# teticio/audio-diffusion

Hardware: NVIDIA H100
Metric: mel-spectrograms/sec (1000-step DDPM, 256x256x1) (higher is better)
Workload: dtype bf16 operands, fp32 accumulate (fp32 master weights, fp64 GroupNorm sums)

## Files before the change

### audio_diffusion_b200/csrc/conv_tc.cu

```cuda
#include <cuda.h>
#include <cudaTypedefs.h>

#include <cstdlib>

#include "conv_tc.cuh"

namespace b200ad {

struct alignas(64) ConvMaps {
  CUtensorMap src[CONV_MAXSEG];
  CUtensorMap out;
};

__host__ __device__ __forceinline__ int window_pixels(const ConvParams& p, const ConvSeg& sg, int G) {
  return p.tile2d ? (p.tw + sg.hl + sg.hr) * (p.th + sg.ht + sg.hb)
                  : G * CONV_TM + (sg.ht + sg.hb) * p.Wp + sg.hl + sg.hr;
}
__host__ __device__ __forceinline__ int window_pitch(const ConvParams& p, const ConvSeg& sg) {
  return p.tile2d ? p.tw + sg.hl + sg.hr : p.Wp;
}

constexpr int CONV_THREADS = 384;
constexpr int CONV_XF_THREADS = 64;
constexpr int CONV_SPLANE = CONV_MAXG * CONV_TM * 16;
constexpr int CONV_STG_WG = 8 * CONV_SPLANE;
constexpr int CONV_STAGING = 2 * CONV_STG_WG;
static size_t conv_smem_bytes(const ConvParams& p) {
  return (size_t)p.as * p.a_stage + (size_t)p.bs * CONV_B_SLOT + CONV_STAGING + 1024;
}

struct WorkItem {
  int n, ntile, m0, G;
  int r0, c0;
};

__device__ __forceinline__ WorkItem decode_work(const ConvParams& p, int w) {
  WorkItem wi;
  wi.ntile = w % p.ntiles_n;
  const int gidx = w / p.ntiles_n;
  if (p.tile2d) {
    wi.n = gidx / p.groups_per_img;
    const int t = gidx - wi.n * p.groups_per_img, tx = t / p.tiles_y;
    wi.r0 = (t - tx * p.tiles_y) * p.th;
    wi.c0 = tx * p.tw;
    wi.m0 = 0;
    wi.G = CONV_MAXG;
    return wi;
  }
  wi.r0 = wi.c0 = 0;
  if (p.pack) {
    wi.n = gidx * p.pack;
    wi.m0 = 0;
    wi.G = min(p.pack, p.N - wi.n);
    return wi;
  }
  wi.n = gidx / p.groups_per_img;
  const int g = gidx - wi.n * p.groups_per_img;
  wi.m0 = g * (CONV_MAXG * CONV_TM);
  const int rem = p.H * p.Wp - wi.m0;
  wi.G = min(CONV_MAXG, (rem + CONV_TM - 1) / CONV_TM);
  return wi;
}

template <bool SILU>
__device__ __forceinline__ uint4 xform_vec(uint4 v, const f32x2_t (&sc)[4], const f32x2_t (&sh)[4]) {
  uint32_t u[4] = {v.x, v.y, v.z, v.w};
#pragma unroll
  for (int e = 0; e < 4; ++e) {
    f32x2_t a = f2_fma(f2_from_bf16x2(u[e]), sc[e], sh[e]);
    if (SILU) {
      const float2 f = f2_unpack(a);
      a = f2_fma(a, f2_pack(tanh_approx(f.x), tanh_approx(f.y)), a);
    }
    u[e] = f2_to_bf16x2(a);
  }
  return make_uint4(u[0], u[1], u[2], u[3]);
}

template <bool SQUARE>
__global__ void __launch_bounds__(CONV_THREADS, 1) conv_tc_kernel(const __grid_constant__ ConvParams p,
                                                                  const __grid_constant__ ConvMaps maps) {
  constexpr int ASM = CONV_AS_MAX, BSM = CONV_BS_MAX;
  const int AS = p.as;
  const int BS = p.bs;
  extern __shared__ __align__(128) uint8_t smem[];
  const int warp = __shfl_sync(0xffffffffu, (int)(threadIdx.x >> 5), 0);
  const int lane = threadIdx.x & 31;
  const int a_bytes = p.a_stage;

  uint8_t* bring = smem + AS * a_bytes;
  uint8_t* stg = bring + BS * CONV_B_SLOT;
  uint8_t* ctrl = stg + CONV_STAGING;
  uint64_t* bars = reinterpret_cast<uint64_t*>(ctrl);
  const uint32_t smem_base = smem_u32(smem);
  const uint32_t bring_base = smem_u32(bring);
  const uint32_t bar_fullA = smem_u32(bars);
  const uint32_t bar_readyA = smem_u32(bars + ASM);
  const uint32_t bar_emptyA = smem_u32(bars + 2 * ASM);
  const uint32_t bar_fullB = smem_u32(bars + 3 * ASM);
  const uint32_t bar_emptyB = smem_u32(bars + 3 * ASM + BSM);
  static_assert((3 * ASM + 2 * BSM) * 8 <= 1024, "barrier block overflows");

  if (warp == 1 && lane == 0) {
    for (int s = 0; s < AS; ++s) {
      mbar_init(bar_fullA + 8 * s, 1);
      mbar_init(bar_readyA + 8 * s, CONV_XF_THREADS / 32);
      mbar_init(bar_emptyA + 8 * s, 8);
    }
    for (int s = 0; s < BS; ++s) {
      mbar_init(bar_fullB + 8 * s, 1);
      mbar_init(bar_emptyB + 8 * s, 8);
    }
    mbar_fence_init();
  }
  __syncthreads();

  asm volatile("griddepcontrol.launch_dependents;" ::: "memory");
  if (warp != 1) asm volatile("griddepcontrol.wait;" ::: "memory");

  if (warp == 0) {
    int stage = 0;
    uint32_t phase = 0;
    for (int w = blockIdx.x; w < p.total_work; w += gridDim.x) {
      const WorkItem wi = decode_work(p, w);
      for (int s = 0; s < p.nseg; ++s) {
        const ConvSeg& sg = p.seg[s];
        const uint32_t row_bytes = (uint32_t)window_pixels(p, sg, wi.G) * 16u;
        for (int ks = 0; ks < sg.ksteps; ++ks) {
          const uint32_t full = bar_fullA + 8 * stage;
          if (lane == 0) {
            mbar_wait(bar_emptyA + 8 * stage, phase ^ 1);
            mbar_arrive_expect_tx(full, 2u * row_bytes);
          }
          __syncwarp();
          const long long plane = (long long)(2 * ks + (lane & 1)) * p.PL;
          if (p.tile2d) {
            if (lane == 0)
              tensor_g2s_4d(smem_base + stage * a_bytes, &maps.src[s], 8 * (wi.c0 - sg.hl), wi.r0 - sg.ht, 2 * ks, wi.n, full);
          } else if (!p.pack) {
            const int pix0 = p.lead + wi.m0 - sg.ht * p.Wp - sg.hl;
            if (lane < 2)
              bulk_g2s(smem_base + stage * a_bytes + (uint32_t)lane * row_bytes,
                       sg.src + (long long)wi.n * sg.img_stride + (plane + pix0) * 8, row_bytes, full);
          } else {
            const int g = lane >> 1, lead_px = sg.ht * p.Wp + sg.hl, trail_px = sg.hb * p.Wp + sg.hr;
            const int cnt = CONV_TM + (g == 0 ? lead_px : 0) + (g == wi.G - 1 ? trail_px : 0);
            const int doff = (g == 0) ? 0 : lead_px + g * CONV_TM;
            const int pix0 = p.lead - (g == 0 ? lead_px : 0);
            if (g < wi.G && lane < 2 * CONV_MAXG)
              bulk_g2s(smem_base + stage * a_bytes + (uint32_t)(lane & 1) * row_bytes + (uint32_t)doff * 16u,
                       sg.src + (long long)(wi.n + g) * sg.img_stride + (plane + pix0) * 8, (uint32_t)cnt * 16u, full);
          }
          if (++stage == AS) { stage = 0; phase ^= 1; }
        }
      }
    }
  } else if (warp == 1) {
    if (lane == 0) {
      int stage = 0;
      uint32_t phase = 0;
      for (int w = blockIdx.x; w < p.total_work; w += gridDim.x) {
        const int ntile = w % p.ntiles_n;
        for (int s = 0; s < p.nseg; ++s) {
          const ConvSeg& sg = p.seg[s];
          const char* src = reinterpret_cast<const char*>(sg.wpack + (long long)ntile * sg.wtile_stride);
          for (int ks = 0; ks < sg.ksteps; ++ks) {
            for (int t0 = 0; t0 < sg.ntaps; t0 += CONV_BT) {
              const uint32_t bytes = (uint32_t)min(CONV_BT, sg.ntaps - t0) * CONV_B_TAP;
              mbar_wait(bar_emptyB + 8 * stage, phase ^ 1);
              if (p.dbg & 32) {
                mbar_arrive(bar_fullB + 8 * stage);
              } else {
                mbar_arrive_expect_tx(bar_fullB + 8 * stage, bytes);
                bulk_g2s(bring_base + stage * CONV_B_SLOT, src, bytes, bar_fullB + 8 * stage);
              }
              src += bytes;
              if (++stage == BS) { stage = 0; phase ^= 1; }
            }
          }
        }
      }
    }
  } else if (warp >= 4) {
    const int cw = (warp - 4) >> 2, wq = warp & 3, tid = threadIdx.x & 127;
    const uint32_t stg_w = smem_u32(stg) + (uint32_t)(cw * CONV_STG_WG);
    const uint32_t st_addr = stg_w + (uint32_t)((2 * wq + ((lane >> 3) & 1)) * CONV_SPLANE + (8 * (lane >> 4) + (lane & 7)) * 16);
    const Geom og = make_geom(p.N, p.up2 ? 2 * p.H : p.H, p.up2 ? 2 * p.W : p.W);
    const long long out_img_stride = (long long)(p.cout >> 3) * og.PL * 8;
    const int hw_end = p.H * p.Wp;
    const bool do_stats = p.stats != nullptr;
    const bool issuer = tid < 8 * CONV_MAXG;
    float acc[CONV_MAXG * CONV_TM / 2];
    int sa = 0, sb = 0;
    uint32_t pa = 0, pb = 0;
    for (int w = blockIdx.x; w < p.total_work; w += gridDim.x) {
      const WorkItem wi = decode_work(p, w);
#pragma unroll
      for (int i = 0; i < CONV_MAXG * CONV_TM / 2; ++i) acc[i] = 0.f;
      int pend_b = -1, pend_a = -1;
      auto release = [&]() {
        __syncwarp();
        if (lane == 0) {
          if (pend_b >= 0) mbar_arrive(bar_emptyB + 8 * pend_b);
          if (pend_a >= 0) mbar_arrive(bar_emptyA + 8 * pend_a);
        }
      };
      for (int s = 0, ks = 0; s < p.nseg;) {
        const ConvSeg& sg = p.seg[s];
        const uint32_t xlbo = (uint32_t)window_pixels(p, sg, wi.G) * 16u;
        const uint32_t xsbo = p.tile2d ? (uint32_t)window_pitch(p, sg) * 16u : 128u;
        const int ntaps = sg.ntaps;
        mbar_wait(bar_readyA + 8 * sa, pa);
        const uint32_t abase = smem_base + sa * a_bytes;
        for (int t0 = 0; t0 < ntaps; t0 += CONV_BT) {
          mbar_wait(bar_fullB + 8 * sb, pb);
          const uint32_t bbase = bring_base + sb * CONV_B_SLOT + (uint32_t)(cw * 1024);
          const int nt = min(CONV_BT, ntaps - t0);
          wgmma_fence();
          for (int t = 0; t < nt; ++t) {
            const uint64_t wdesc = gmma_desc(bbase + (uint32_t)t * CONV_B_TAP, (CONV_NT / 8) * 128, 128);
            const uint64_t xdesc = gmma_desc(abase + (uint32_t)sg.aoff[t0 + t] * 16u, xlbo, xsbo);
            if constexpr (SQUARE) {
              wgmma_m64n128k16_x2(acc, wdesc, xdesc, xdesc + (128u >> 4));
            } else if (wi.G == 2) {
              wgmma_m64n256k16<0, 0>(acc, wdesc, xdesc);
            } else {
              wgmma_m64n128k16<0, 0>(acc, wdesc, xdesc);
            }
          }
          wgmma_commit();
          wgmma_wait<1>();
          release();
          pend_b = sb;
          pend_a = (t0 + CONV_BT >= ntaps) ? sa : -1;
          if (++sb == BS) { sb = 0; pb ^= 1; }
        }
        if (++sa == AS) { sa = 0; pa ^= 1; }
        if (++ks == sg.ksteps) { ks = 0; ++s; }
      }
      wgmma_wait<0>();
      release();

      if (issuer) bulk_wait_read_all();
      named_bar_sync(1 + cw, 128);
      if (!(p.dbg & 8)) {
        float ssum[2] = {0.f, 0.f}, ssq[2] = {0.f, 0.f};
#pragma unroll
        for (int g = 0; g < CONV_MAXG; ++g) {
          if (g < wi.G) {
            const int n = p.pack ? wi.n + g : wi.n;
            float bias[2];
#pragma unroll
            for (int h = 0; h < 2; ++h) {
              const int c = wi.ntile * CONV_NT + cw * 64 + wq * 16 + 8 * h + (lane >> 2);
              bias[h] = p.bias ? __ldg(p.bias + c) : 0.f;
              if (p.temb) bias[h] += __ldg(p.temb + (long long)n * p.temb_stride + c);
            }
            int m = (p.pack ? 0 : wi.m0 + g * CONV_TM) + 2 * (lane & 3);
            int col = m % p.Wp;
#pragma unroll
            for (int k = 0; k < CONV_TM / 16; ++k) {
              uint32_t pk[4];
#pragma unroll
              for (int u = 0; u < 2; ++u) {
                const int col1 = (col + 1 == p.Wp) ? 0 : col + 1;
                const bool v0 = p.tile2d || (m < hw_end && col < p.W), v1 = p.tile2d || (m + 1 < hw_end && col1 < p.W);
#pragma unroll
                for (int h = 0; h < 2; ++h) {
                  const int j = g * (CONV_TM / 8) + 2 * k + u;
                  const float a0 = v0 ? acc[4 * j + 2 * h] + bias[h] : 0.f;
                  const float a1 = v1 ? acc[4 * j + 2 * h + 1] + bias[h] : 0.f;
                  ssum[h] += a0 + a1;
                  ssq[h] = fmaf(a0, a0, fmaf(a1, a1, ssq[h]));
                  pk[2 * u + h] = pack_bf16x2(a0, a1);
                }
                m += 8;
                col += 8;
                while (col >= p.Wp) col -= p.Wp;
              }
              stmatrix_x4_trans(st_addr + (uint32_t)((g * CONV_TM + 16 * k) * 16), pk[0], pk[1], pk[2], pk[3]);
            }
            if (do_stats && (p.pack || g == wi.G - 1)) {
#pragma unroll
              for (int h = 0; h < 2; ++h) {
                float s1 = ssum[h], s2 = ssq[h];
#pragma unroll
                for (int o = 1; o < 16; o <<= 1) {
                  s1 += __shfl_xor_sync(0xffffffffu, s1, o);
                  s2 += __shfl_xor_sync(0xffffffffu, s2, o);
                }
                if ((lane & 15) == 0) {
                  const int c = wi.ntile * CONV_NT + cw * 64 + wq * 16 + 8 * h + (lane >> 2);
                  stat_t* sdst = p.stats + ((long long)n * (p.cout >> 2) + (c >> 2)) * 2;
                  atomicAdd(sdst, (stat_t)s1);
                  atomicAdd(sdst + 1, (stat_t)s2);
                }
                ssum[h] = 0.f;
                ssq[h] = 0.f;
              }
            }
          }
        }
      }
      if (p.tile2d) {
        fence_proxy_async_smem();
        named_bar_sync(1 + cw, 128);
        if (SQUARE) {
          const int g = tid >> 3, pl = tid & 7;
          if (issuer && !(p.dbg & 2)) {
            const uint32_t src = stg_w + (uint32_t)(pl * CONV_SPLANE + g * CONV_TM * 16);
            const int c = wi.c0 + 8 * g, plane = wi.ntile * 16 + cw * 8 + pl;
            if (p.up2) tensor_s2g_5d(&maps.out, 0, c, wi.r0, plane, wi.n, src);
            else       tensor_s2g_4d(&maps.out, 8 * c, wi.r0, plane, wi.n, src);
            bulk_commit();
          }
        } else if (tid == 0 && !(p.dbg & 2)) {
          tensor_s2g_4d(&maps.out, 8 * wi.c0, wi.r0, wi.ntile * 16 + cw * 8, wi.n, stg_w);
          bulk_commit();
        }
      } else if (!p.up2) {
        fence_proxy_async_smem();
        named_bar_sync(1 + cw, 128);
        const int g = tid >> 3, pl = tid & 7;
        if (issuer && g < wi.G && !(p.dbg & 2)) {
          const int n = p.pack ? wi.n + g : wi.n;
          bulk_s2g(p.out + (long long)n * out_img_stride + (long long)(wi.ntile * 16 + cw * 8 + pl) * og.PL * 8 +
                       (long long)(p.lead + (p.pack ? 0 : wi.m0 + CONV_TM * g)) * 8,
                   stg_w + (uint32_t)(pl * CONV_SPLANE + g * CONV_TM * 16), (uint32_t)CONV_TM * 16u);
          bulk_commit();
        }
      } else {
        named_bar_sync(1 + cw, 128);
        const int npx = wi.G * CONV_TM;
        for (int i = tid; i < 8 * npx && !(p.dbg & 2); i += 128) {
          const int pl = i / npx, px = i - pl * npx, g = px >> 7;
          const int m = p.pack ? px & (CONV_TM - 1) : wi.m0 + px;
          const int hh = m / p.Wp, ww = m - hh * p.Wp;
          if (m < hw_end && ww < p.W) {
            const int n = p.pack ? wi.n + g : wi.n;
            const uint4 o = *reinterpret_cast<const uint4*>(stg + cw * CONV_STG_WG + pl * CONV_SPLANE + px * 16);
            *reinterpret_cast<uint4*>(p.out + (long long)n * out_img_stride + (long long)(wi.ntile * 16 + cw * 8 + pl) * og.PL * 8 +
                                      (long long)(og.lead + (2 * hh + p.oy) * og.Wp + 2 * ww + p.ox) * 8) = o;
          }
        }
      }
    }
    if (issuer) bulk_wait_all();
  } else {
    const int tidx = (warp - 2) * 32 + lane;
    int stage = 0;
    uint32_t phase = 0;
    for (int w = blockIdx.x; w < p.total_work; w += gridDim.x) {
      const WorkItem wi = decode_work(p, w);
      for (int s = 0; s < p.nseg; ++s) {
        const ConvSeg& sg = p.seg[s];
        const int npix = window_pixels(p, sg, wi.G);
        const int pitch = window_pitch(p, sg);
        const float2* ssn = sg.ss ? sg.ss + (long long)wi.n * sg.ss_stride : nullptr;
        const int cbase = p.tile2d ? wi.c0 - sg.hl : 0;
        int row0, col0;
        if (p.tile2d) {
          row0 = wi.r0 - sg.ht + tidx / pitch;
          col0 = tidx - (tidx / pitch) * pitch;
        } else {
          const int m_first = wi.m0 - sg.ht * p.Wp - sg.hl + tidx;
          row0 = (m_first >= 0) ? m_first / p.Wp : -1 - ((-1 - m_first) / p.Wp);
          col0 = m_first - row0 * p.Wp;
        }
        const int drow = CONV_XF_THREADS / pitch;
        const int dcol = CONV_XF_THREADS - drow * pitch;
        const bool silu = sg.silu != 0;
        for (int ks = 0; ks < sg.ksteps; ++ks) {
          f32x2_t sc0[4], sh0[4], sc1[4], sh1[4];
          if (ssn && !p.pack) {
            const float4* sp = reinterpret_cast<const float4*>(ssn + ks * 16);
            const float hs = silu ? 0.5f : 1.0f;
#pragma unroll
            for (int e = 0; e < 4; ++e) {
              const float4 a = __ldg(sp + e), b = __ldg(sp + 4 + e);
              sc0[e] = f2_pack(a.x * hs, a.z * hs); sh0[e] = f2_pack(a.y * hs, a.w * hs);
              sc1[e] = f2_pack(b.x * hs, b.z * hs); sh1[e] = f2_pack(b.y * hs, b.w * hs);
            }
          }
          mbar_wait(bar_fullA + 8 * stage, phase);
          if (ssn && p.pack && !(p.dbg & 64)) {
            uint4* base = reinterpret_cast<uint4*>(smem + stage * a_bytes);
            const int lead_px = sg.ht * p.Wp + sg.hl, hw = p.H * p.Wp;
            const float hs = silu ? 0.5f : 1.0f;
            for (int g = 0; g < wi.G; ++g) {
              const float4* sp = reinterpret_cast<const float4*>(ssn + (long long)g * sg.ss_stride + ks * 16);
#pragma unroll
              for (int e = 0; e < 4; ++e) {
                const float4 a = __ldg(sp + e), b = __ldg(sp + 4 + e);
                sc0[e] = f2_pack(a.x * hs, a.z * hs); sh0[e] = f2_pack(a.y * hs, a.w * hs);
                sc1[e] = f2_pack(b.x * hs, b.z * hs); sh1[e] = f2_pack(b.y * hs, b.w * hs);
              }
              for (int m = tidx; m < hw; m += CONV_XF_THREADS) {
                const int r = m / p.Wp;
                const int px = lead_px + g * CONV_TM + m;
                uint4 a = make_uint4(0, 0, 0, 0), b = make_uint4(0, 0, 0, 0);
                if (m - r * p.Wp < p.W) {
                  a = base[px];
                  b = base[npix + px];
                  if (silu) { a = xform_vec<true>(a, sc0, sh0); b = xform_vec<true>(b, sc1, sh1); }
                  else      { a = xform_vec<false>(a, sc0, sh0); b = xform_vec<false>(b, sc1, sh1); }
                }
                base[px] = a;
                base[npix + px] = b;
              }
            }
            fence_proxy_async_smem();
          } else if (ssn && !(p.dbg & 64)) {
            uint4* base = reinterpret_cast<uint4*>(smem + stage * a_bytes);
            int row = row0, col = col0;
            for (int px = tidx; px < npix; px += CONV_XF_THREADS) {
              const bool valid = (row >= 0) && (row < p.H) && ((unsigned)(cbase + col) < (unsigned)p.W);
              uint4 a = make_uint4(0, 0, 0, 0), b = make_uint4(0, 0, 0, 0);
              if (valid) {
                a = base[px];
                b = base[npix + px];
                if (silu) { a = xform_vec<true>(a, sc0, sh0); b = xform_vec<true>(b, sc1, sh1); }
                else      { a = xform_vec<false>(a, sc0, sh0); b = xform_vec<false>(b, sc1, sh1); }
              }
              base[px] = a;
              base[npix + px] = b;
              row += drow; col += dcol;
              if (col >= pitch) { col -= pitch; ++row; }
            }
            fence_proxy_async_smem();
          }
          __syncwarp();
          if (lane == 0) mbar_arrive(bar_readyA + 8 * stage);
          if (++stage == AS) { stage = 0; phase ^= 1; }
        }
      }
    }
  }

  if (p.fin.ss) __threadfence();
  __syncthreads();

  if (p.fin.ss) {
    __shared__ unsigned s_last;
    if (threadIdx.x == 0) {
      __threadfence();
      s_last = (atomicAdd(p.fin.counter, 1u) == gridDim.x - 1) ? 1u : 0u;
    }
    __syncthreads();
    if (s_last) {
      __threadfence();
      const ConvGnFin& f = p.fin;
      const int Ct = f.C[0] + f.C[1], cpg = Ct / f.groups;
      float* gmean = reinterpret_cast<float*>(smem);
      float* grstd = gmean + p.N * f.groups;
      const double cnt = (double)cpg * (double)f.HW;
      for (int i = threadIdx.x; i < p.N * f.groups; i += CONV_THREADS) {
        const int n = i / f.groups, gi = i - n * f.groups;
        double sm = 0., sq = 0.;
        for (int c0 = gi * cpg; c0 < (gi + 1) * cpg; c0 += 32) {
          double2 v[8];
#pragma unroll
          for (int k = 0; k < 8; ++k) {
            const int c = c0 + 4 * k;
            v[k] = make_double2(0., 0.);
            if (c < (gi + 1) * cpg) {
              const stat_t* st = (c < f.C[0]) ? f.stats[0] + ((long long)n * (f.C[0] >> 2) + (c >> 2)) * 2
                                              : f.stats[1] + ((long long)n * (f.C[1] >> 2) + ((c - f.C[0]) >> 2)) * 2;
              v[k] = __ldcg(reinterpret_cast<const double2*>(st));
            }
          }
#pragma unroll
          for (int k = 0; k < 8; ++k) { sm += v[k].x; sq += v[k].y; }
        }
        const double mean = sm / cnt;
        gmean[i] = (float)mean;
        grstd[i] = (float)(1.0 / sqrt(fmax(sq / cnt - mean * mean, 0.) + (double)f.eps));
      }
      __syncthreads();
      {
        const int total = p.N * Ct;
        const int dn = CONV_THREADS / Ct, dc = CONV_THREADS - dn * Ct;
        const float inv_cpg = 1.0f / (float)cpg;
        int i = threadIdx.x;
        int n = i / Ct, c = i - n * Ct;
        for (; i < total; i += CONV_THREADS) {
          const int gi = n * f.groups + (int)(((float)c + 0.5f) * inv_cpg);
          const float sc = __ldg(f.gamma + c) * grstd[gi];
          f.ss[i] = make_float2(sc, __ldg(f.beta + c) - gmean[gi] * sc);
          n += dn;
          c += dc;
          if (c >= Ct) { c -= Ct; ++n; }
        }
      }
      if (threadIdx.x == 0) *f.counter = 0u;
    }
  }
}

static cudaError_t encode_pf8_map(CUtensorMap* m, const __nv_bfloat16* base, const ConvParams& p, int cs, int rs, long long pl,
                                  int planes, long long img_stride, int bw, int bh, int bplanes) {
  static PFN_cuTensorMapEncodeTiled_v12000 encode = nullptr;
  if (!encode) {
    void* fn = nullptr;
    cudaDriverEntryPointQueryResult q;
    cudaError_t e = cudaGetDriverEntryPointByVersion("cuTensorMapEncodeTiled", &fn, 12000, cudaEnableDefault, &q);
    if (e != cudaSuccess) return e;
    if (q != cudaDriverEntryPointSuccess || !fn) return cudaErrorNotSupported;
    encode = reinterpret_cast<PFN_cuTensorMapEncodeTiled_v12000>(fn);
  }
  const cuuint32_t estride[5] = {1, 1, 1, 1, 1};
  CUresult r;
  if (cs == 1) {
    const cuuint64_t dim[4] = {(cuuint64_t)p.W * 8, (cuuint64_t)p.H, (cuuint64_t)planes, (cuuint64_t)p.N};
    const cuuint64_t stride[3] = {(cuuint64_t)rs * 16, (cuuint64_t)pl * 16, (cuuint64_t)img_stride * 2};
    const cuuint32_t box[4] = {(cuuint32_t)bw * 8, (cuuint32_t)bh, (cuuint32_t)bplanes, 1};
    r = encode(m, CU_TENSOR_MAP_DATA_TYPE_BFLOAT16, 4, (void*)base, dim, stride, box, estride, CU_TENSOR_MAP_INTERLEAVE_NONE,
               CU_TENSOR_MAP_SWIZZLE_NONE, CU_TENSOR_MAP_L2_PROMOTION_L2_256B, CU_TENSOR_MAP_FLOAT_OOB_FILL_NONE);
  } else {
    const cuuint64_t dim[5] = {8, (cuuint64_t)p.W, (cuuint64_t)p.H, (cuuint64_t)planes, (cuuint64_t)p.N};
    const cuuint64_t stride[4] = {(cuuint64_t)cs * 16, (cuuint64_t)rs * 16, (cuuint64_t)pl * 16, (cuuint64_t)img_stride * 2};
    const cuuint32_t box[5] = {8, (cuuint32_t)bw, (cuuint32_t)bh, (cuuint32_t)bplanes, 1};
    r = encode(m, CU_TENSOR_MAP_DATA_TYPE_BFLOAT16, 5, (void*)base, dim, stride, box, estride, CU_TENSOR_MAP_INTERLEAVE_NONE,
               CU_TENSOR_MAP_SWIZZLE_NONE, CU_TENSOR_MAP_L2_PROMOTION_L2_256B, CU_TENSOR_MAP_FLOAT_OOB_FILL_NONE);
  }
  return r == CUDA_SUCCESS ? cudaSuccess : cudaErrorInvalidValue;
}

int conv_dbg_env() {
  const char* dbg_env = getenv("B200AD_CONV_DBG");
  return dbg_env ? atoi(dbg_env) : 0;
}

cudaError_t plan_conv_tc(ConvParams& p, int num_sms) {
  if (p.nseg < 1 || p.nseg > CONV_MAXSEG) return cudaErrorInvalidValue;
  for (int s = 0; s < p.nseg; ++s) {
    ConvSeg& sg = p.seg[s];
    if (sg.ntaps > CONV_MAXTAPS || sg.ksteps < 1) return cudaErrorInvalidValue;
    if (sg.wtile_stride == 0) sg.wtile_stride = (long long)sg.ksteps * sg.ntaps * (CONV_B_TAP / 2);
    sg.ht = sg.hb = sg.hl = sg.hr = 0;
    for (int t = 0; t < sg.ntaps; ++t) {
      sg.ht |= sg.dh[t] < 0; sg.hb |= sg.dh[t] > 0;
      sg.hl |= sg.dw[t] < 0; sg.hr |= sg.dw[t] > 0;
    }
  }
  p.tile2d = 0;
  p.tw = p.th = 0;
  p.tiles_y = 0;
  p.groups_per_img = (p.H * p.Wp + CONV_MAXG * CONV_TM - 1) / (CONV_MAXG * CONV_TM);
  p.ntiles_n = p.cout / CONV_NT;
  p.total_work = p.N * p.groups_per_img * p.ntiles_n;
  p.pack = 0;
  int fits = 1;
  for (int s = 0; s < p.nseg; ++s) {
    const ConvSeg& sg = p.seg[s];
    if (p.H * p.Wp + sg.hb * p.Wp + sg.hr > CONV_TM || sg.ht * p.Wp + sg.hl > CONV_TM) fits = 0;
  }
  if (fits) {
    int best = 1;
    long long best_cost = -1;
    for (int g = 1; g <= CONV_MAXG; g *= 2) {
      const long long items = (long long)((p.N + g - 1) / g) * p.ntiles_n;
      const long long cost = ((items + num_sms - 1) / num_sms) * g;
      if (best_cost < 0 || cost <= best_cost) { best_cost = cost; best = g; }
    }
    p.pack = best;
    p.total_work = ((p.N + best - 1) / best) * p.ntiles_n;
  }
  const int tiles_img = (p.H * p.Wp + CONV_TM - 1) / CONV_TM;
  const int max_g = p.pack ? p.pack : (tiles_img < CONV_MAXG ? tiles_img : CONV_MAXG);
  if (!p.pack && !(p.dbg & 4096)) {
    auto window_cost = [&](const ConvParams& q, int G) {
      long long c = 0;
      for (int s = 0; s < q.nseg; ++s) c += (long long)window_pixels(q, q.seg[s], G) * q.seg[s].ksteps;
      return c;
    };
    long long best[3] = {(long long)tiles_img * CONV_TM, p.groups_per_img, 0};
    for (int i = 0; i < p.groups_per_img; ++i) best[2] += window_cost(p, min(CONV_MAXG, tiles_img - CONV_MAXG * i));
    const int shapes[2][2] = {{8, 32}, {16, 16}};
    for (const auto& sh : shapes) {
      const int tw = sh[0], th = sh[1];
      if (p.W % tw || p.H % th) continue;
      if (tw == 16 && p.H >= 64 && p.H % 32 == 0 && p.W % 8 == 0) continue;
      if (tw == 8 && p.up2) continue;
      ConvParams q = p;
      q.tile2d = 1; q.tw = tw; q.th = th;
      const long long items = (long long)(p.W / tw) * (p.H / th);
      const long long c[3] = {items * CONV_MAXG * CONV_TM, items, items * window_cost(q, CONV_MAXG)};
      if (c[0] < best[0] || (c[0] == best[0] && (c[1] < best[1] || (c[1] == best[1] && c[2] < best[2])))) {
        best[0] = c[0]; best[1] = c[1]; best[2] = c[2];
        p.tile2d = 1; p.tw = tw; p.th = th;
      }
    }
    if (p.tile2d) {
      p.tiles_y = p.H / p.th;
      p.groups_per_img = (p.W / p.tw) * p.tiles_y;
      p.total_work = p.N * p.groups_per_img * p.ntiles_n;
    }
  }
  int a_stage = 0;
  for (int s = 0; s < p.nseg; ++s) {
    const ConvSeg& sg = p.seg[s];
    const int npix = window_pixels(p, sg, max_g), pitch = window_pitch(p, sg);
    a_stage = npix * 32 > a_stage ? npix * 32 : a_stage;
    if (sg.ntaps > CONV_MAXTAPS || sg.ntaps > CONV_BT * (CONV_BS - 1) || npix > 0x3FFF) return cudaErrorInvalidValue;
    for (int t = 0; t < sg.ntaps; ++t) p.seg[s].aoff[t] = (sg.dh[t] + sg.ht) * pitch + sg.dw[t] + sg.hl;
  }
  p.a_stage = (a_stage + 255) & ~255;
  p.as = CONV_AS;
  p.bs = CONV_BS;
  auto rings_fit = [&](int as, int bs) {
    return (size_t)as * p.a_stage + (size_t)bs * CONV_B_SLOT + CONV_STAGING + 2048 <= (size_t)CONV_SMEM_MAX;
  };
  while (p.as < 6 && rings_fit(p.as + 1, p.bs)) ++p.as;
  while (p.bs < CONV_BS_MAX && rings_fit(p.as, p.bs + 1)) ++p.bs;
  while (p.as < CONV_AS_MAX && rings_fit(p.as + 1, p.bs)) ++p.as;
  if (conv_smem_bytes(p) > (size_t)CONV_SMEM_MAX) return cudaErrorInvalidValue;
  return cudaSuccess;
}

cudaError_t launch_conv_tc(const ConvParams& p_in, int num_sms, cudaStream_t stream) {
  ConvParams p = p_in;
  p.dbg = conv_dbg_env();
  if (cudaError_t e = plan_conv_tc(p, num_sms)) return e;
  ConvMaps maps{};
  if (p.tile2d) {
    for (int s = 0; s < p.nseg; ++s) {
      const ConvSeg& sg = p.seg[s];
      cudaError_t e = encode_pf8_map(&maps.src[s], sg.src + (long long)p.lead * 8, p, 1, p.Wp, p.PL, 2 * sg.ksteps,
                                     sg.img_stride, p.tw + sg.hl + sg.hr, p.th + sg.ht + sg.hb, 2);
      if (e != cudaSuccess) return e;
    }
    const int bh = p.th, bplanes = p.tw == 16 ? 1 : 8;
    cudaError_t e;
    if (p.up2) {
      const Geom og = make_geom(p.N, 2 * p.H, 2 * p.W);
      e = encode_pf8_map(&maps.out, p.out + (long long)(og.lead + p.oy * og.Wp + p.ox) * 8, p, 2, 2 * og.Wp, og.PL,
                         p.cout / 8, (long long)(p.cout / 8) * og.PL * 8, 8, bh, bplanes);
    } else {
      e = encode_pf8_map(&maps.out, p.out + (long long)p.lead * 8, p, 1, p.Wp, p.PL, p.cout / 8,
                         (long long)(p.cout / 8) * p.PL * 8, 8, bh, bplanes);
    }
    if (e != cudaSuccess) return e;
  }
  const size_t smem = conv_smem_bytes(p);
  const int grid = p.total_work < num_sms ? p.total_work : num_sms;
  if (grid <= 0) return cudaSuccess;
  const bool square = p.tile2d && p.tw == 16;
  void (*kernel)(ConvParams, ConvMaps) = square ? conv_tc_kernel<true> : conv_tc_kernel<false>;
  static size_t attr[2] = {0, 0};
  if (smem > attr[square]) {
    cudaError_t e = cudaFuncSetAttribute(kernel, cudaFuncAttributeMaxDynamicSharedMemorySize, (int)smem);
    if (e != cudaSuccess) return e;
    attr[square] = smem;
  }
  cudaLaunchConfig_t cfg = {};
  cfg.gridDim = dim3((unsigned)grid);
  cfg.blockDim = dim3(CONV_THREADS);
  cfg.dynamicSmemBytes = smem;
  cfg.stream = stream;
  cudaLaunchAttribute at[1];
  at[0].id = cudaLaunchAttributeProgrammaticStreamSerialization;
  at[0].val.programmaticStreamSerializationAllowed = 1;
  cfg.attrs = at;
  cfg.numAttrs = 1;
  return cudaLaunchKernelEx(&cfg, kernel, p, maps);
}

__global__ void pack_identity_kernel(int channels, __nv_bfloat16* __restrict__ dst, long long nvec) {
  const long long id = (long long)blockIdx.x * blockDim.x + threadIdx.x;
  if (id >= nvec) return;
  const int r = (int)(id & 7), n8 = (int)((id >> 3) & 15), k8 = (int)((id >> 7) & 1);
  const long long rest = id >> 8;
  const int ksteps = channels / 16;
  const int ks = (int)(rest % ksteps), ntile = (int)(rest / ksteps);
  const int co = ntile * 128 + n8 * 8 + r;
  const int ci0 = ks * 16 + k8 * 8;
  uint32_t o[4];
#pragma unroll
  for (int e = 0; e < 4; ++e) o[e] = pack_bf16x2(co == ci0 + 2 * e ? 1.f : 0.f, co == ci0 + 2 * e + 1 ? 1.f : 0.f);
  reinterpret_cast<uint4*>(dst)[id] = make_uint4(o[0], o[1], o[2], o[3]);
}
cudaError_t launch_pack_identity(int channels, __nv_bfloat16* dst, cudaStream_t s) {
  const long long nvec = (long long)(channels / 128) * (channels / 16) * 256;
  pack_identity_kernel<<<(unsigned)((nvec + 255) / 256), 256, 0, s>>>(channels, dst, nvec);
  return cudaGetLastError();
}

}
```

Before: 0.9318.

## Specialize conv kernel on tile shape and preload bias into accumulators

The conv kernel now has three compile-time shape variants (flat, 8x32 tiled, 16x16 tiled), so the tile2d branches, validity checks and column tracking fold away in the tiled epilogues. Bias plus time-embedding is also loaded for the next work item while the current epilogue runs and is used to initialise the wgmma accumulators. This removes the per-element bias add and the dependent global loads from the epilogue. The cost is an extra kernel instantiation and more registers held for the prefetched bias values.

Measured after the change: 0.9453 (median of 6 runs). 1.4% higher.

```diff
diff --git a/audio_diffusion_b200/csrc/conv_tc.cu b/audio_diffusion_b200/csrc/conv_tc.cu
--- a/audio_diffusion_b200/csrc/conv_tc.cu
+++ b/audio_diffusion_b200/csrc/conv_tc.cu
@@ -34,11 +34,14 @@
   int r0, c0;
 };
 
+enum ConvShape { CONV_FLAT = 0, CONV_T8X32 = 1, CONV_T16X16 = 2 };
+
+template <int SHAPE>
 __device__ __forceinline__ WorkItem decode_work(const ConvParams& p, int w) {
   WorkItem wi;
   wi.ntile = w % p.ntiles_n;
   const int gidx = w / p.ntiles_n;
-  if (p.tile2d) {
+  if constexpr (SHAPE != CONV_FLAT) {
     wi.n = gidx / p.groups_per_img;
     const int t = gidx - wi.n * p.groups_per_img, tx = t / p.tiles_y;
     wi.r0 = (t - tx * p.tiles_y) * p.th;
@@ -77,9 +80,10 @@
   return make_uint4(u[0], u[1], u[2], u[3]);
 }
 
-template <bool SQUARE>
+template <int SHAPE>
 __global__ void __launch_bounds__(CONV_THREADS, 1) conv_tc_kernel(const __grid_constant__ ConvParams p,
                                                                   const __grid_constant__ ConvMaps maps) {
+  constexpr bool TILED = SHAPE != CONV_FLAT, SQUARE = SHAPE == CONV_T16X16;
   constexpr int ASM = CONV_AS_MAX, BSM = CONV_BS_MAX;
   const int AS = p.as;
   const int BS = p.bs;
@@ -122,7 +126,7 @@
     int stage = 0;
     uint32_t phase = 0;
     for (int w = blockIdx.x; w < p.total_work; w += gridDim.x) {
-      const WorkItem wi = decode_work(p, w);
+      const WorkItem wi = decode_work<SHAPE>(p, w);
       for (int s = 0; s < p.nseg; ++s) {
         const ConvSeg& sg = p.seg[s];
         const uint32_t row_bytes = (uint32_t)window_pixels(p, sg, wi.G) * 16u;
@@ -190,13 +194,33 @@
     const int hw_end = p.H * p.Wp;
     const bool do_stats = p.stats != nullptr;
     const bool issuer = tid < 8 * CONV_MAXG;
+    const int chan = cw * 64 + wq * 16 + (lane >> 2);
+    float b0[CONV_MAXG][2];
+    auto load_bias = [&](int w) {
+      const WorkItem wi = decode_work<SHAPE>(p, w);
+#pragma unroll
+      for (int h = 0; h < 2; ++h) {
+        const int c = wi.ntile * CONV_NT + chan + 8 * h;
+        const float b = p.bias ? __ldg(p.bias + c) : 0.f;
+#pragma unroll
+        for (int g = 0; g < CONV_MAXG; ++g) {
+          if (g == 0 || (!TILED && p.pack)) {
+            const int n = min(wi.n + g, p.N - 1);
+            b0[g][h] = p.temb ? b + __ldg(p.temb + (long long)n * p.temb_stride + c) : b;
+          } else {
+            b0[g][h] = b0[0][h];
+          }
+        }
+      }
+    };
+    if (blockIdx.x < p.total_work) load_bias(blockIdx.x);
     float acc[CONV_MAXG * CONV_TM / 2];
     int sa = 0, sb = 0;
     uint32_t pa = 0, pb = 0;
     for (int w = blockIdx.x; w < p.total_work; w += gridDim.x) {
-      const WorkItem wi = decode_work(p, w);
-#pragma unroll
-      for (int i = 0; i < CONV_MAXG * CONV_TM / 2; ++i) acc[i] = 0.f;
+      const WorkItem wi = decode_work<SHAPE>(p, w);
+#pragma unroll
+      for (int i = 0; i < CONV_MAXG * CONV_TM / 2; ++i) acc[i] = b0[i / (CONV_TM / 2)][(i >> 1) & 1];
       int pend_b = -1, pend_a = -1;
       auto release = [&]() {
         __syncwarp();
@@ -208,7 +232,7 @@
       for (int s = 0, ks = 0; s < p.nseg;) {
         const ConvSeg& sg = p.seg[s];
         const uint32_t xlbo = (uint32_t)window_pixels(p, sg, wi.G) * 16u;
-        const uint32_t xsbo = p.tile2d ? (uint32_t)window_pitch(p, sg) * 16u : 128u;
+        const uint32_t xsbo = TILED ? (uint32_t)window_pitch(p, sg) * 16u : 128u;
         const int ntaps = sg.ntaps;
         mbar_wait(bar_readyA + 8 * sa, pa);
         const uint32_t abase = smem_base + sa * a_bytes;
@@ -222,6 +246,8 @@
             const uint64_t xdesc = gmma_desc(abase + (uint32_t)sg.aoff[t0 + t] * 16u, xlbo, xsbo);
             if constexpr (SQUARE) {
               wgmma_m64n128k16_x2(acc, wdesc, xdesc, xdesc + (128u >> 4));
+            } else if constexpr (TILED) {
+              wgmma_m64n256k16<0, 0>(acc, wdesc, xdesc);
             } else if (wi.G == 2) {
               wgmma_m64n256k16<0, 0>(acc, wdesc, xdesc);
             } else {
@@ -240,6 +266,7 @@
       }
       wgmma_wait<0>();
       release();
+      if (w + (int)gridDim.x < p.total_work) load_bias(w + gridDim.x);
 
       if (issuer) bulk_wait_read_all();
       named_bar_sync(1 + cw, 128);
@@ -247,40 +274,41 @@
         float ssum[2] = {0.f, 0.f}, ssq[2] = {0.f, 0.f};
 #pragma unroll
         for (int g = 0; g < CONV_MAXG; ++g) {
-          if (g < wi.G) {
-            const int n = p.pack ? wi.n + g : wi.n;
-            float bias[2];
-#pragma unroll
-            for (int h = 0; h < 2; ++h) {
-              const int c = wi.ntile * CONV_NT + cw * 64 + wq * 16 + 8 * h + (lane >> 2);
-              bias[h] = p.bias ? __ldg(p.bias + c) : 0.f;
-              if (p.temb) bias[h] += __ldg(p.temb + (long long)n * p.temb_stride + c);
-            }
-            int m = (p.pack ? 0 : wi.m0 + g * CONV_TM) + 2 * (lane & 3);
-            int col = m % p.Wp;
+          if (TILED || g < wi.G) {
+            const bool pack = !TILED && p.pack;
+            const int n = pack ? wi.n + g : wi.n;
+            int m = 0, col = 0;
+            if constexpr (!TILED) {
+              m = (pack ? 0 : wi.m0 + g * CONV_TM) + 2 * (lane & 3);
+              col = m % p.Wp;
+            }
 #pragma unroll
             for (int k = 0; k < CONV_TM / 16; ++k) {
               uint32_t pk[4];
 #pragma unroll
               for (int u = 0; u < 2; ++u) {
-                const int col1 = (col + 1 == p.Wp) ? 0 : col + 1;
-                const bool v0 = p.tile2d || (m < hw_end && col < p.W), v1 = p.tile2d || (m + 1 < hw_end && col1 < p.W);
+                bool v0 = true, v1 = true;
+                if constexpr (!TILED) {
+                  const int col1 = (col + 1 == p.Wp) ? 0 : col + 1;
+                  v0 = m < hw_end && col < p.W;
+                  v1 = m + 1 < hw_end && col1 < p.W;
+                  m += 8;
+                  col += 8;
+                  while (col >= p.Wp) col -= p.Wp;
+                }
 #pragma unroll
                 for (int h = 0; h < 2; ++h) {
                   const int j = g * (CONV_TM / 8) + 2 * k + u;
-                  const float a0 = v0 ? acc[4 * j + 2 * h] + bias[h] : 0.f;
-                  const float a1 = v1 ? acc[4 * j + 2 * h + 1] + bias[h] : 0.f;
+                  const float a0 = v0 ? acc[4 * j + 2 * h] : 0.f;
+                  const float a1 = v1 ? acc[4 * j + 2 * h + 1] : 0.f;
                   ssum[h] += a0 + a1;
                   ssq[h] = fmaf(a0, a0, fmaf(a1, a1, ssq[h]));
                   pk[2 * u + h] = pack_bf16x2(a0, a1);
                 }
-                m += 8;
-                col += 8;
-                while (col >= p.Wp) col -= p.Wp;
               }
               stmatrix_x4_trans(st_addr + (uint32_t)((g * CONV_TM + 16 * k) * 16), pk[0], pk[1], pk[2], pk[3]);
             }
-            if (do_stats && (p.pack || g == wi.G - 1)) {
+            if (do_stats && (pack || g == (TILED ? CONV_MAXG : wi.G) - 1)) {
 #pragma unroll
               for (int h = 0; h < 2; ++h) {
                 float s1 = ssum[h], s2 = ssq[h];
@@ -290,7 +318,7 @@
                   s2 += __shfl_xor_sync(0xffffffffu, s2, o);
                 }
                 if ((lane & 15) == 0) {
-                  const int c = wi.ntile * CONV_NT + cw * 64 + wq * 16 + 8 * h + (lane >> 2);
+                  const int c = wi.ntile * CONV_NT + chan + 8 * h;
                   stat_t* sdst = p.stats + ((long long)n * (p.cout >> 2) + (c >> 2)) * 2;
                   atomicAdd(sdst, (stat_t)s1);
                   atomicAdd(sdst + 1, (stat_t)s2);
@@ -302,10 +330,10 @@
           }
         }
       }
-      if (p.tile2d) {
+      if constexpr (TILED) {
         fence_proxy_async_smem();
         named_bar_sync(1 + cw, 128);
-        if (SQUARE) {
+        if constexpr (SQUARE) {
           const int g = tid >> 3, pl = tid & 7;
           if (issuer && !(p.dbg & 2)) {
             const uint32_t src = stg_w + (uint32_t)(pl * CONV_SPLANE + g * CONV_TM * 16);
@@ -351,7 +379,7 @@
     int stage = 0;
     uint32_t phase = 0;
     for (int w = blockIdx.x; w < p.total_work; w += gridDim.x) {
-      const WorkItem wi = decode_work(p, w);
+      const WorkItem wi = decode_work<SHAPE>(p, w);
       for (int s = 0; s < p.nseg; ++s) {
         const ConvSeg& sg = p.seg[s];
         const int npix = window_pixels(p, sg, wi.G);
@@ -645,13 +673,15 @@
   const size_t smem = conv_smem_bytes(p);
   const int grid = p.total_work < num_sms ? p.total_work : num_sms;
   if (grid <= 0) return cudaSuccess;
-  const bool square = p.tile2d && p.tw == 16;
-  void (*kernel)(ConvParams, ConvMaps) = square ? conv_tc_kernel<true> : conv_tc_kernel<false>;
-  static size_t attr[2] = {0, 0};
-  if (smem > attr[square]) {
+  const int shape = !p.tile2d ? CONV_FLAT : p.tw == 16 ? CONV_T16X16 : CONV_T8X32;
+  void (*const kernels[3])(ConvParams, ConvMaps) = {conv_tc_kernel<CONV_FLAT>, conv_tc_kernel<CONV_T8X32>,
+                                                    conv_tc_kernel<CONV_T16X16>};
+  void (*kernel)(ConvParams, ConvMaps) = kernels[shape];
+  static size_t attr[3] = {0, 0, 0};
+  if (smem > attr[shape]) {
     cudaError_t e = cudaFuncSetAttribute(kernel, cudaFuncAttributeMaxDynamicSharedMemorySize, (int)smem);
     if (e != cudaSuccess) return e;
-    attr[square] = smem;
+    attr[shape] = smem;
   }
   cudaLaunchConfig_t cfg = {};
   cfg.gridDim = dim3((unsigned)grid);
```
